# Danderson123/Amira

Hardware: AMD Instinct MI355X
Metric: gene-mers/s to corrected GeneMerGraph (higher is better)
Workload: dtype int32; 1 GPU; synthetic 1M reads x 60 genes, k=5, 20k-gene vocab: build + error-correction sweep (build, filter(3,1), correct, build, clip(5), correct, build); reads_per_gpu=1000000, genes_per_read=60, k=5, vocab=20000, gene_mers_per_gpu=56000000, final_nodes=472478, final_edges=1054844, multi_gpu=n/a

## Files before the change

amira_amd/csrc/amg_build_x.hip:

```cpp
#include "amg_tile.h"
#include "amg_x.h"

template <class View>
__device__ __forceinline__ void x_fp94(const View& w, int k, int flip, int dir, unsigned long long seed, int weak,
                                       unsigned long long& w1, unsigned int& tag) {
  unsigned long long h1 = seed, h2 = seed ^ 0xC2B2AE3D27D4EB4Full;
  for (int j = 0; j < k; ++j) {
    const unsigned long long c = (unsigned long long)(unsigned int)canon_tok(w, k, flip, dir, j);
    h1 = (h1 ^ c) * 0x9E3779B97F4A7C15ull;
    h1 ^= h1 >> 29;
    h2 = (h2 + c) * 0xD6E8FEB86659FD93ull;
    h2 ^= h2 >> 31;
  }
  h1 = mix64(h1);
  h2 = mix64(h2 ^ (h1 >> 7));
  if (weak) {
    h1 &= 0xfffull;
    h2 = 0ull;
  }
  w1 = (h1 << 1) | 1ull;
  tag = ((unsigned int)h2 << 1) | 1u;
}

__global__ __launch_bounds__(256) void k_x_verify_fp(const int* __restrict__ tokens, long long n_tokens, int k, int flip,
// ... 229 lines not shown

#define FD_READS 16
__global__ __launch_bounds__(256) void k_x_flag_dead_reads(const int* __restrict__ tok_node,
                                                            const long long* __restrict__ read_off, long long n_reads,
                                                            unsigned char* __restrict__ read_fix) {
  const int lane = threadIdx.x & 63, sub = lane & 15, grp = lane >> 4;
  const long long r = ((long long)blockIdx.x * 4 + (threadIdx.x >> 6)) * 4 + grp;
  const bool have = r < n_reads;
  const long long a = have ? read_off[r] : 0, b = have ? read_off[r + 1] : 0;
  int v[4];
#pragma unroll
  for (int j = 0; j < 4; ++j) v[j] = a + sub + 16 * j < b ? tok_node[a + sub + 16 * j] : 0;
  bool hit = v[0] == -2 || v[1] == -2 || v[2] == -2 || v[3] == -2;
  for (long long t = a + 64 + sub; t < b; t += 16) hit = hit || (tok_node[t] == -2);
  const unsigned long long m = __ballot(hit);
  if (have && sub == 0 && ((m >> (grp * 16)) & 0xffffull)) read_fix[r] = 1;
}

__global__ void k_x_rank_setflags(const unsigned int* __restrict__ first2, long long n, int shift,
                                  unsigned char* __restrict__ flags) {
  long long i = (long long)blockIdx.x * blockDim.x + threadIdx.x;
  if (i >= n) return;
  const unsigned int fi = x_first_inv(first2, i);
  if (fi == 0u) return;
  flags[(~fi) >> shift] = 1;
}

__device__ __forceinline__ long long x_rank_of(unsigned int t, const unsigned int* __restrict__ bits,
                                               const long long* __restrict__ prefix) {
  const unsigned int w = bits[t >> 5];
  return prefix[t >> 5] + (long long)__popc(w & ((1u << (t & 31)) - 1u));
}

__global__ void k_x_assign_nodes_ranked(const unsigned int* __restrict__ first2, long long n_nodes,
                                        const unsigned int* __restrict__ bits, const long long* __restrict__ prefix,
                                        const Slot16* __restrict__ tab, const unsigned int* __restrict__ slot_by_claim,
                                        int k, int nbits, int two, int* __restrict__ final_of_claim,
                                        int* __restrict__ node_tokens, long long* __restrict__ node_first,
                                        unsigned char* __restrict__ node_alive, const int* __restrict__ tokens, int flip) {
  long long c = (long long)blockIdx.x * blockDim.x + threadIdx.x;
  if (c >= n_nodes) return;
  if (x_first_inv(first2, c) == 0u) return;
  const unsigned int first = ~x_first_inv(first2, c);
  const long long i = x_rank_of(first >> 1, bits, prefix);
  final_of_claim[c] = (int)i;
  node_first[i] = (long long)first;
  node_alive[i] = 1;
  if (nbits == 0) {
    const long long f = (long long)(first >> 1);
    for (int j = 0; j < k; ++j) node_tokens[i * k + j] = (first & 1u) ? flip - tokens[f + k - 1 - j] : tokens[f + j];
    return;
  }
  const Slot16 s = tab[slot_by_claim[c]];
  const unsigned int tag = two ? (unsigned int)(s.w2 >> 32) : 0u;
  for (int j = 0; j < k; ++j) node_tokens[i * k + j] = x_unpack(s.w1, tag, nbits, j);
}

__device__ __forceinline__ void pair_to_final(unsigned long long& key, unsigned int& first,
                                              const int* __restrict__ fin) {
  const unsigned int lo_c = (unsigned int)((key >> 32) & 0x7fffffffull);
  const unsigned int hi_c = (unsigned int)(key & 0xffffffffull) - 1u;
  const bool a_is_lo = (first & 1u) != 0u;
  const unsigned int X = (unsigned int)fin[a_is_lo ? lo_c : hi_c], Y = (unsigned int)fin[a_is_lo ? hi_c : lo_c];
  const unsigned int lo = X < Y ? X : Y, hi = X < Y ? Y : X;
  key = (key & (1ull << 63)) | ((unsigned long long)lo << 32) | (unsigned long long)(hi + 1u);
  first = (first & ~1u) | (X == lo ? 1u : 0u);
}

__global__ void k_x_gather_pairs_ranked(const unsigned int* __restrict__ first2, long long n_pairs,
                                        const unsigned int* __restrict__ bits, const long long* __restrict__ prefix,
                                        const Slot16* __restrict__ etab, const unsigned int* __restrict__ slot_by_claim,
                                        const unsigned int* __restrict__ cnt_by_claim,
                                        unsigned long long* __restrict__ pkey, unsigned long long* __restrict__ pfirst,
                                        unsigned int* __restrict__ pcnt, const int* __restrict__ fin,
                                        int* __restrict__ efinal) {
  long long c = (long long)blockIdx.x * blockDim.x + threadIdx.x;
  if (c >= n_pairs) return;
  if (x_first_inv(first2, c) == 0u) return;
  unsigned int first = ~x_first_inv(first2, c);
  const long long i = x_rank_of(first >> 3, bits, prefix);
  unsigned long long key = etab[slot_by_claim[c]].w1;
  if (fin) pair_to_final(key, first, fin);
  pkey[i] = key;
  pfirst[i] = (unsigned long long)first;
  if (efinal)
    efinal[c] = (int)i;
  else
    pcnt[i] = cnt_by_claim[c];
}

__global__ void k_x_sort_keys(const unsigned int* __restrict__ first2, long long n,
                              unsigned int* __restrict__ keys, unsigned int* __restrict__ vals) {
  long long i = (long long)blockIdx.x * blockDim.x + threadIdx.x;
  if (i >= n) return;
  keys[i] = ~x_first_inv(first2, i);
  vals[i] = (unsigned int)i;
}

__global__ void k_x_assign_nodes(const unsigned int* __restrict__ first_sorted,
                                 const unsigned int* __restrict__ claim_sorted, long long n_nodes,
                                 const Slot16* __restrict__ tab, const unsigned int* __restrict__ slot_by_claim,
                                 int k, int bits, int two, int* __restrict__ final_of_claim,
                                 int* __restrict__ node_tokens, long long* __restrict__ node_first,
                                 unsigned char* __restrict__ node_alive, const int* __restrict__ tokens, int flip) {
  long long i = (long long)blockIdx.x * blockDim.x + threadIdx.x;
  if (i >= n_nodes) return;
  const unsigned int c = claim_sorted[i];
  final_of_claim[c] = (int)i;
  node_first[i] = (long long)first_sorted[i];
  node_alive[i] = 1;
  if (bits == 0) {
    const unsigned int first = first_sorted[i];
    const long long f = (long long)(first >> 1);
    for (int j = 0; j < k; ++j) node_tokens[i * k + j] = (first & 1u) ? flip - tokens[f + k - 1 - j] : tokens[f + j];
    return;
  }
  const Slot16 s = tab[slot_by_claim[c]];
  const unsigned int tag = two ? (unsigned int)(s.w2 >> 32) : 0u;
  for (int j = 0; j < k; ++j) node_tokens[i * k + j] = x_unpack(s.w1, tag, bits, j);
}

__global__ void k_xc_init(int* parent, long long n) {
  long long i = (long long)blockIdx.x * blockDim.x + threadIdx.x;
  if (i < n) parent[i] = (int)i;
}

__global__ void k_xc_union(const int* __restrict__ tok_claim, long long n_tokens, int* parent) {
  long long t = (long long)blockIdx.x * blockDim.x + threadIdx.x;
  if (t + 1 >= n_tokens) return;
  const int raw = tok_claim[t];
  if (raw == -1 || ((unsigned int)raw & AMG_LAST_FLAG)) return;
  const int nxt = tok_claim[t + 1];
  if (nxt == -1) return;
  int a = (int)((unsigned int)raw & ~AMG_FLAG_MASK), b = (int)((unsigned int)nxt & ~AMG_FLAG_MASK);
  while (true) {
    a = uf_find(parent, a);
    b = uf_find(parent, b);
    if (a == b) break;
    if (a > b) { int x = a; a = b; b = x; }
    const int old = atomicCAS(parent + b, b, a);
    if (old == b) break;
    b = old;
  }
}

__global__ void k_xc_flatten(int* parent, long long n) {
  long long i = (long long)blockIdx.x * blockDim.x + threadIdx.x;
  if (i < n) parent[i] = uf_find(parent, (int)i);
}

__device__ __forceinline__ int xc_root(const int* __restrict__ parent, long long c) {
  int r = parent[c];
// ... 428 lines not shown
    unsigned long long v[2] = {0, 0};
    AMGCHK(fetch(c, l, v));
    D = v[0];
    if (v[1]) {
      stage_end(c);
      return overflowed(which, OV_COLLISION);
    }
  }
  stage_end(c);
  c->n_nodes = (int64_t)D;
  AMGCHK(bx_nodes_rank(c));
  if (n > 0 && D > 0)
    hipLaunchKernelGGL(k_x_cov_from_claims, dim3(nblk(n, 256)), dim3(256), 0, st, c->x_ecnt.as<unsigned int>(),
                       c->x_first.as<unsigned int>(), c->x_final.as<int>(), n, c->node_cov.as<unsigned int>(), (int*)nullptr);
  return AMG_OK;
}

int bx_nodes_rank(amg_ctx* c) {
  hipStream_t st = c->stream;
  const long long T = c->n_tokens;
  const int k = c->k;
  stage_begin(c, "node_rank");
  const long long D = c->n_nodes;
  AMGCHK(c->s1.ensure((size_t)(D + 1) * sizeof(unsigned int)));
  AMGCHK(c->s2.ensure((size_t)(D + 1) * sizeof(unsigned int)));
  AMGCHK(c->s3.ensure((size_t)(D + 1) * sizeof(unsigned int)));
  AMGCHK(c->s4.ensure((size_t)(D + 1) * sizeof(unsigned int)));
  AMGCHK(bs_alloc_nodes(c, D));
  const long long S = c->x_nspace;
  if (D > 0 && ((D <= kRankBitmapMax && !c->sw.rank_sort) || S != D)) {
    AMGCHK(x_rank_bitmap(c, c->x_first.as<unsigned int>(), S, 1));
    hipLaunchKernelGGL(k_x_assign_nodes_ranked, dim3(nblk(S, 256)), dim3(256), 0, st,
                       c->x_first.as<unsigned int>(), S,
                       c->s1.as<unsigned int>(), c->s5.as<long long>(), c->node_tab.as<Slot16>(),
                       c->x_slot.as<unsigned int>(), k, c->x_kbits, c->x_two ? 1 : 0,
                       c->x_final.as<int>(), c->node_tokens.as<int>(),
                       c->node_first.as<long long>(), c->node_alive.as<unsigned char>(), c->tokens.as<int>(), c->two_v - 1);
  } else if (D > 0) {
    c->rank_flags_clean = 0;
    hipLaunchKernelGGL(k_x_sort_keys, dim3(nblk(D, 256)), dim3(256), 0, st, c->x_first.as<unsigned int>(),
                       D, c->s1.as<unsigned int>(),
                       c->s3.as<unsigned int>());
    AMGCHK(prim_sort_u32_u32(c, c->s1.as<unsigned int>(), c->s2.as<unsigned int>(), c->s3.as<unsigned int>(),
                             c->s4.as<unsigned int>(), (size_t)D, ilog2_ceil((uint64_t)T * 2 + 2) + 1));
    hipLaunchKernelGGL(k_x_assign_nodes, dim3(nblk(D, 256)), dim3(256), 0, st, c->s2.as<unsigned int>(),
                       c->s4.as<unsigned int>(), D, c->node_tab.as<Slot16>(), c->x_slot.as<unsigned int>(),
                       k, c->x_kbits, c->x_two ? 1 : 0, c->x_final.as<int>(),
                       c->node_tokens.as<int>(), c->node_first.as<long long>(), c->node_alive.as<unsigned char>(),
                       c->tokens.as<int>(), c->two_v - 1);
  }
  stage_end(c);
  return AMG_OK;
}

int bx_edges(amg_ctx* c, Overflow* which, unsigned int min_edge_cov) {
  bool lone = false;
  if (min_edge_cov == 0) {
    const bool can = c->sw.edge_home && c->n_nodes > 0;
    lone = can && (c->sw.edge_lone >= 0 ? c->sw.edge_lone != 0 : c->n_nodes * 16 > c->n_tokens);
    AMGCHK(bx_node_count(c, lone));
  }
  AMGCHK(bx_edges_upsert(c, which, lone, min_edge_cov == 0));
  return bx_edges_rank(c, min_edge_cov, min_edge_cov == 0);
}

int bx_node_count(amg_ctx* c, bool tag) {
  const long long T = c->n_tokens, D = c->n_nodes;
  stage_begin(c, "node_count");
  const long long S = c->x_nspace;
  AMGCHK(c->x_ncnt.ensure((size_t)(S + 2) * sizeof(unsigned int)));
  if (tag) AMGCHK(c->x_ftag.ensure((size_t)(S + 2) * sizeof(int)));
  AMGCHK(count_ids(c, CountNodes, IdsClaimsMarked, c->tok_slot.as<int>(), T, S, c->x_ncnt.as<unsigned int>()));
  if (S > 0 && D > 0)
    hipLaunchKernelGGL(k_x_cov_from_claims, dim3(nblk(S, 256)), dim3(256), 0, c->stream,
                       c->x_ncnt.as<unsigned int>(), c->x_first.as<unsigned int>(), c->x_final.as<int>(), S,
                       c->node_cov.as<unsigned int>(), tag ? c->x_ftag.as<int>() : (int*)nullptr);
  stage_end(c);
  return AMG_OK;
}

// ... 150 lines not shown
```

amira_amd/csrc/amg_filter.hip:

```cpp
#include "amg_rows.h"

__global__ void k_filter_nodes(const unsigned int* __restrict__ cov, unsigned char* __restrict__ alive,
                               long long n, unsigned int min_cov) {
  long long i = (long long)blockIdx.x * blockDim.x + threadIdx.x;
  if (i < n && alive[i] && cov[i] < min_cov) alive[i] = 0;
}

__global__ void k_filter_edges(const int* __restrict__ src, const int* __restrict__ tgt,
                               const unsigned int* __restrict__ cov,
                               const unsigned char* __restrict__ node_alive,
                               unsigned char* __restrict__ alive, long long n, unsigned int min_cov) {
  long long e = (long long)blockIdx.x * blockDim.x + threadIdx.x;
  if (e >= n || !alive[e]) return;
  if ((min_cov > 1 && cov[e] < min_cov) || !node_alive[src[e]] || !node_alive[tgt[e]]) alive[e] = 0;
}

#define READS_PER_WAVE 8
__global__ __launch_bounds__(256) void k_mask_reads(int* __restrict__ tok_node,
                                                    const long long* __restrict__ read_off,
                                                    long long n_reads,
                                                    const unsigned char* __restrict__ node_alive,
                                                    unsigned char* __restrict__ read_fix) {
  const long long rbase = ((long long)blockIdx.x * 4 + (threadIdx.x >> 6)) * READS_PER_WAVE;
  if (rbase >= n_reads) return;
  const int lane = threadIdx.x & 63;
  const long long off_l = (lane <= READS_PER_WAVE && rbase + lane <= n_reads) ? read_off[rbase + lane] : 0;
  long long a[READS_PER_WAVE], b[READS_PER_WAVE];
  int v[READS_PER_WAVE];
#pragma unroll
  for (int j = 0; j < READS_PER_WAVE; ++j) {
    a[j] = __shfl(off_l, j, 64);
    b[j] = rbase + j < n_reads ? __shfl(off_l, j + 1, 64) : a[j];
  }
#pragma unroll
  for (int j = 0; j < READS_PER_WAVE; ++j) v[j] = a[j] + lane < b[j] ? tok_node[a[j] + lane] : -1;
  bool dead[READS_PER_WAVE];
#pragma unroll
  for (int j = 0; j < READS_PER_WAVE; ++j) dead[j] = v[j] >= 0 && !node_alive[v[j]];
#pragma unroll
  for (int j = 0; j < READS_PER_WAVE; ++j) {
    if (dead[j]) tok_node[a[j] + lane] = -2;
    bool hit = dead[j];
    for (long long t = a[j] + 64 + lane; t < b[j]; t += 64) {
      const int n = tok_node[t];
      if (n >= 0 && !node_alive[n]) {
        tok_node[t] = -2;
        hit = true;
      }
    }
    if (__any(hit) && lane == 0) read_fix[rbase + j] = 1;
  }
}

static int apply_removals(amg_ctx* c, unsigned int min_edge_cov) {
  hipStream_t st = c->stream;
  if (min_edge_cov > 1) live_lists_after_edge_deaths(c);
  else live_lists_after_node_deaths(c);
  if (c->n_edges > 0)
    hipLaunchKernelGGL(k_filter_edges, dim3(nblk(c->n_edges, 256)), dim3(256), 0, st,
                       c->edge_src.as<int>(), c->edge_tgt.as<int>(), c->edge_cov.as<unsigned int>(),
                       c->node_alive.as<unsigned char>(), c->edge_alive.as<unsigned char>(),
                       c->n_edges, min_edge_cov);
  if (c->n_reads > 0)
    hipLaunchKernelGGL(k_mask_reads, dim3(nblk(c->n_reads, 4 * READS_PER_WAVE)), dim3(256), 0, st,
                       c->tok_node.as<int>(), c->read_off.as<long long>(), c->n_reads,
                       c->node_alive.as<unsigned char>(), c->read_fix.as<unsigned char>());
  return AMG_OK;
}

extern "C" int amg_filter(amg_ctx* c, uint32_t min_node_cov, uint32_t min_edge_cov) {
  NEED_BUILT(c);
  stages_reset(c);
  stage_begin(c, "filter");
  if (c->n_nodes > 0)
    hipLaunchKernelGGL(k_filter_nodes, dim3(nblk(c->n_nodes, 256)), dim3(256), 0, c->stream,
                       c->node_cov.as<unsigned int>(), c->node_alive.as<unsigned char>(),
                       c->n_nodes, min_node_cov);
  AMGCHK(apply_removals(c, min_edge_cov));
  stage_end(c);
  c->have_corrected = false;
  return AMG_OK;
}

__global__ void k_kill_listed(const int* __restrict__ ids, long long n, long long n_nodes,
                              unsigned char* __restrict__ alive) {
  long long i = (long long)blockIdx.x * blockDim.x + threadIdx.x;
  if (i >= n) return;
  int v = ids[i];
  if (v >= 0 && v < n_nodes) alive[v] = 0;
}

extern "C" int amg_remove_nodes(amg_ctx* c, const int32_t* node_ids, int64_t n) {
// ... 283 lines not shown
```

amira_amd/csrc/amg_internal.h:

```cpp
#pragma once
#include <cstdint>
#include <cstdio>
#include <cstring>
#include <string>
#include <vector>

#include <hip/hip_runtime.h>

#include "amg_host.h"

#define HIPCHK(call)                                                                   \
  do {                                                                                 \
    hipError_t e_ = (call);                                                            \
    if (e_ != hipSuccess)                                                              \
      return amg_fail(AMG_E_HIP, "%s:%d %s -> %s", __FILE__, __LINE__, #call,          \
                      hipGetErrorString(e_));                                          \
  } while (0)
#define AMGCHK(call)                 \
  do {                               \
    int r_ = (call);                 \
    if (r_ != AMG_OK) return r_;     \
  } while (0)

struct DevBuf {
// ... 255 lines not shown

  BuildSwitches sw;
  std::vector<StageTime> stages;
  bool timing = true;
};

struct amg_seqs {
  int device = 0;
  DevBuf bases, off;
  int64_t n = 0, total = 0;
};

int prim_sort_u64_u32(amg_ctx* c, const unsigned long long* kin, unsigned long long* kout,
                      const unsigned int* vin, unsigned int* vout, size_t n, int end_bit);
int prim_sort_u32_u32(amg_ctx* c, const unsigned int* kin, unsigned int* kout,
                      const unsigned int* vin, unsigned int* vout, size_t n, int end_bit);
struct ClearList;
int prim_exscan_i64(amg_ctx* c, const long long* in, long long* out, size_t n);
int prim_exscan_u32_to_i64(amg_ctx* c, const unsigned int* in, long long* out, size_t n);
int prim_exscan_u32_pair(amg_ctx* c, const unsigned int* in_a, long long* out_a, const unsigned int* in_b, long long* out_b,
                         size_t n);
int prim_exscan_i64_pair(amg_ctx* c, const long long* in_a, long long* out_a, const long long* in_b, long long* out_b,
                         size_t n);
int prim_exscan_bytes_set(amg_ctx* c, const unsigned char* in, long long* out, size_t n, const ClearList* side = nullptr);
int prim_exscan_apply_kill(amg_ctx* c, unsigned char* kill, unsigned char* alive, long long* out, size_t n);
int prim_exscan_keep_and_len(amg_ctx* c, const unsigned int* len, long long* out_keep, long long* out_off, size_t n);
int prim_exscan_flag_words(amg_ctx* c, const unsigned char* flags, unsigned int* bits, long long* out, size_t n_words);
int prim_exscan_bits_popc(amg_ctx* c, const unsigned int* bits, long long* out, size_t n_words);
int prim_exscan_pair_width(amg_ctx* c, const unsigned long long* pkey, long long* out, size_t n_pairs);
int prim_exscan_emit_edges(amg_ctx* c, const unsigned long long* pkey, const unsigned int* pcnt,
                           const unsigned long long* pfirst, size_t n_pairs, long long* total, int* e_src, int* e_tgt,
                           signed char* e_sdir, signed char* e_tdir, unsigned int* e_cov, unsigned char* e_alive,
                           const ClearList* side);

#define CLEAR_MAX 8
struct ClearList {
  void* p[CLEAR_MAX];
  unsigned long long bytes[CLEAR_MAX];
  int n = 0;
  bool overflow = false;
  unsigned int fill[CLEAR_MAX];
  void add(void* ptr, size_t b, unsigned int value = 0u) {
    if (b == 0) return;
    if (n >= CLEAR_MAX) {
      overflow = true;
      return;
    }
    p[n] = ptr;
    bytes[n] = (unsigned long long)((b + 3) & ~(size_t)3);
    fill[n] = value;
    ++n;
  }
};
int clear_many(amg_ctx* c, const ClearList& l);

#define FETCH_MAX 96
struct FetchList {
  const unsigned long long* p[FETCH_MAX];
  int n = 0;
  bool overflow = false;
  void add(const void* q) {
    if (n < FETCH_MAX)
      p[n++] = static_cast<const unsigned long long*>(q);
    else
      overflow = true;
  }
// ... 96 lines not shown
```

amira_amd/csrc/amg_live_rows.hip:

```cpp
#include "amg_rows.h"

void live_lists_after_node_deaths(amg_ctx* c) {
  if (c->live_lists == LiveLists::Current)
    c->live_lists = getenv("AMG_NO_LADJ_PATCH") ? LiveLists::Absent : LiveLists::BehindNodes;
  c->pristine = false;
  c->match_valid = false;
}

void live_lists_after_edge_deaths(amg_ctx* c) {
  c->live_lists = LiveLists::Absent;
  c->edge_own_deaths = true;
  c->pristine = false;
  c->match_valid = false;
}

void live_lists_after_build(amg_ctx* c) { c->live_lists = LiveLists::Absent; }

__global__ void k_live_keys(const unsigned char* __restrict__ e_alive, const int* __restrict__ e_src,
                            const signed char* __restrict__ e_sdir, const long long* __restrict__ pos,
                            long long n_edges, unsigned int* __restrict__ keys, unsigned int* __restrict__ vals) {
  long long e = (long long)blockIdx.x * blockDim.x + threadIdx.x;
  if (e >= n_edges || !e_alive[e]) return;
  const long long o = pos[e];
  keys[o] = adj_row_of(e_src[e], e_sdir[e]);
  vals[o] = (unsigned int)e;
}

__global__ void k_lr_count(const unsigned int* __restrict__ keys, long long n_live, int4* __restrict__ lrows) {
  long long i = (long long)blockIdx.x * blockDim.x + threadIdx.x;
  if (i < n_live) atomicAdd(&lrows[keys[i]].y, 1);
}

#define LR_PER 8
__global__ __launch_bounds__(256) void k_lr_alloc(const unsigned int* __restrict__ keys, long long n_live,
                                                  int4* __restrict__ lrows, unsigned int* __restrict__ tick,
                                                  unsigned long long* pool) {
  __shared__ unsigned int s_wave[4];
  __shared__ unsigned long long s_base;
  const long long i0 = (long long)blockIdx.x * (256 * LR_PER) + threadIdx.x;
  unsigned int cnt[LR_PER], key[LR_PER], mine = 0;
#pragma unroll
  for (int j = 0; j < LR_PER; ++j) {
    const long long i = i0 + (long long)j * 256;
    cnt[j] = 0;
    key[j] = 0;
    if (i < n_live) {
      key[j] = keys[i];
      const unsigned int t = (unsigned int)atomicAdd(&lrows[key[j]].z, 1);
      tick[i] = t;
      if (t == 0) cnt[j] = (unsigned int)lrows[key[j]].y | 0x80000000u;
      mine += cnt[j] & 0x7fffffffu;
    }
  }
  unsigned int total;
  unsigned int off = block_exscan_256(mine, &total, s_wave);
  if (threadIdx.x == 0) s_base = total ? atomicAdd(pool, (unsigned long long)total) : 0ull;
  __syncthreads();
#pragma unroll
  for (int j = 0; j < LR_PER; ++j)
// ... 69 lines not shown
  const int4 rw = lrows[r];
  if (rw.y == 0) return;
  if (!n_alive[r >> 1]) {
    lrows[r] = make_int4(rw.x, 0, 0, 0);
    return;
  }
  if (rw.y == 1) {
    if (!n_alive[rw.z]) lrows[r] = make_int4(rw.x, 0, 0, 0);
    return;
  }
  int w = 0;
  int2 first = make_int2(0, 0);
  for (int j = 0; j < rw.y; ++j) {
    const int2 e = lent[rw.x + j];
    if (!n_alive[e.x]) continue;
    if (w != j) lent[rw.x + w] = e;
    if (w == 0) first = e;
    ++w;
  }
  if (w != rw.y) lrows[r] = make_int4(rw.x, w, first.x, first.y);
}

int ensure_live_adj(amg_ctx* c) {
  if (c->live_lists == LiveLists::Current) return AMG_OK;
  hipStream_t st = c->stream;
  if (c->live_lists == LiveLists::BehindNodes) {
    hipLaunchKernelGGL(k_lr_patch, dim3(nblk(2 * c->n_nodes, 256)), dim3(256), 0, st, c->ladj_rows.as<int4>(),
                       c->ladj.as<int2>(), 2 * c->n_nodes, c->node_alive.as<unsigned char>());
    c->live_lists = LiveLists::Current;
    return AMG_OK;
  }
  const long long rows = 2 * c->n_nodes, E = c->n_edges;
  AMGCHK(c->ladj_rows.ensure((size_t)(rows + 2) * sizeof(int4)));
  AMGCHK(c->ladj_pos.ensure((size_t)(E + 2) * sizeof(long long)));
  unsigned long long* ctr = c->status.as<unsigned long long>() + ST_COMPACT_A;
  {
    ClearList cl;
    cl.add(c->ladj_rows.p, (size_t)(rows + 2) * sizeof(int4));
    cl.add(ctr, 2 * sizeof(unsigned long long));
    AMGCHK(prim_exscan_bytes_set(c, c->edge_alive.as<unsigned char>(), c->ladj_pos.as<long long>(), (size_t)E, &cl));
  }
  long long total = 0;
  {
    FetchList l;
    l.add(c->ladj_pos.as<long long>() + E);
    AMGCHK(fetch(c, l, reinterpret_cast<unsigned long long*>(&total)));
  }
  AMGCHK(c->ladj.ensure((size_t)(total + 1) * sizeof(int2)));
  AMGCHK(c->ladj_keys.ensure(5 * (size_t)(total + 2) * sizeof(unsigned int)));
  unsigned int* keys = c->ladj_keys.as<unsigned int>();
  unsigned int* edge_of = keys + (total + 2);
  unsigned int* tick = edge_of + (total + 2);
  unsigned int* tmp = tick + (total + 2);
  unsigned int* long_rows = tmp + (total + 2);
  if (total > 0) {
    hipLaunchKernelGGL(k_live_keys, dim3(nblk(E, 256)), dim3(256), 0, st, c->edge_alive.as<unsigned char>(),
                       c->edge_src.as<int>(), c->edge_sdir.as<signed char>(), c->ladj_pos.as<long long>(), E, keys,
                       edge_of);
    hipLaunchKernelGGL(k_lr_count, dim3(nblk(total, 256)), dim3(256), 0, st, keys, total, c->ladj_rows.as<int4>());
    hipLaunchKernelGGL(k_lr_alloc, dim3(nblk(total, 256 * LR_PER)), dim3(256), 0, st, keys, total, c->ladj_rows.as<int4>(),
                       tick, ctr);
    hipLaunchKernelGGL(k_lr_fill, dim3(nblk(total, 256)), dim3(256), 0, st, keys, edge_of, tick, total,
                       c->ladj_rows.as<int4>(), c->edge_tgt.as<int>(), c->edge_tdir.as<signed char>(), tmp, c->ladj.as<int2>());
    hipLaunchKernelGGL(k_lr_finish, dim3(nblk(total, 256)), dim3(256), 0, st, keys, tick, total, tmp, c->edge_tgt.as<int>(),
                       c->edge_tdir.as<signed char>(), c->ladj_rows.as<int4>(), c->ladj.as<int2>(), long_rows, ctr + 1);
    const long long hub_words = (E + 31) / 32 + 1;
    AMGCHK(c->hub_bits.ensure((size_t)HUB_BLOCKS * (size_t)hub_words * sizeof(unsigned int)));
    hipLaunchKernelGGL(k_lr_long, dim3(64), dim3(256), 0, st, long_rows, ctr + 1, tmp, c->edge_tgt.as<int>(),
                       c->edge_tdir.as<signed char>(), c->ladj_rows.as<int4>(), c->ladj.as<int2>(),
                       c->hub_bits.as<unsigned int>(), hub_words);
  }
  c->live_lists = LiveLists::Current;
  return AMG_OK;
}

GView make_view(amg_ctx* c) {
  GView g;
  g.lent = c->ladj.as<int2>();
  g.lrows = c->ladj_rows.as<int4>();
  g.n_alive = c->node_alive.as<unsigned char>();
  g.n_cov = c->node_cov.as<unsigned int>();
  g.n_tok = c->node_tokens.as<int>();
  g.n_first = c->node_first.as<long long>();
  g.n_comp = c->node_comp.as<int>();
  g.k = c->k;
  g.flip = c->two_v - 1;
  return g;
}

__global__ void k_row_tickets(const unsigned char* __restrict__ e_alive, const int* __restrict__ e_src,
                              const signed char* __restrict__ e_sdir, long long n_edges, int4* __restrict__ rows) {
// ... 30 lines not shown
```

amira_amd/csrc/amg_scan.hip:

```cpp
#include "amg_device.h"

#define SC_THREADS 512
#define SC_ROWS 16
#define SC_TILE (SC_THREADS * SC_ROWS)
#define SC_VAL_MASK ((1ull << 48) - 1ull)

__device__ __forceinline__ unsigned long long sc_word(unsigned int state, unsigned int epoch, unsigned long long v) {
  return ((unsigned long long)state << 62) | ((unsigned long long)(epoch & 0x3fffu) << 48) | (v & SC_VAL_MASK);
}

#define SC_NO_LIM 0x7fffffffffffffffll
template <class T>
struct LoadArr {
  const T* in;
  using Raw = T;
  __device__ __forceinline__ long long lim() const { return SC_NO_LIM; }
  __device__ __forceinline__ Raw raw(long long i) const { return in[i]; }
  __device__ __forceinline__ unsigned long long val(long long, Raw r) const { return (unsigned long long)r; }
};
template <class T>
struct LoadArrN {
  const T* in;
  long long n;
  using Raw = T;
  __device__ __forceinline__ long long lim() const { return n; }
  __device__ __forceinline__ Raw raw(long long i) const { return in[i]; }
  __device__ __forceinline__ unsigned long long val(long long, Raw r) const { return (unsigned long long)r; }
};
struct LoadNonzero {
  const unsigned int* in;
  long long n;
  using Raw = unsigned int;
  __device__ __forceinline__ long long lim() const { return n; }
// ... 69 lines not shown
struct LoadNone {
  using Raw = unsigned char;
  __device__ __forceinline__ long long lim() const { return 0; }
  __device__ __forceinline__ Raw raw(long long) const { return 0; }
  __device__ __forceinline__ unsigned long long val(long long, Raw) const { return 0ull; }
};

template <class L>
__device__ __forceinline__ void load_rows(const L& ld, long long w0, long long n, int lane, unsigned long long* x) {
  const long long lim = n < ld.lim() ? n : ld.lim();
  if (w0 >= lim) {
#pragma unroll
    for (int r = 0; r < SC_ROWS; ++r) x[r] = 0ull;
    return;
  }
  typename L::Raw raw[SC_ROWS];
#pragma unroll
  for (int r = 0; r < SC_ROWS; ++r) {
    const long long i = w0 + r * 64 + lane;
    raw[r] = ld.raw(i < lim ? i : lim - 1);
  }
  asm volatile("" ::: "memory");
#pragma unroll
  for (int r = 0; r < SC_ROWS; ++r) {
    const long long i = w0 + r * 64 + lane;
    x[r] = i < lim ? ld.val(i, raw[r]) : 0ull;
  }
}

struct EmitOut {
  long long* out;
  struct Pre {};
  __device__ __forceinline__ Pre pre(long long) const { return Pre{}; }
  __device__ __forceinline__ void operator()(long long i, unsigned long long excl, const Pre&) const {
    out[i] = (long long)excl;
  }
};
struct EmitEdges {
  const unsigned long long* pkey;
  const unsigned int* pcnt;
  const unsigned long long* pfirst;
  long long n_pairs;
  long long* total;
  int* e_src;
  int* e_tgt;
  signed char* e_sdir;
  signed char* e_tdir;
  unsigned int* e_cov;
  unsigned char* e_alive;
  struct Pre {
    unsigned long long key, first;
    unsigned int cnt;
  };
  __device__ __forceinline__ Pre pre(long long i) const {
    const long long j = i < n_pairs ? i : 0;
    return Pre{pkey[j], pfirst[j], pcnt[j]};
  }
  __device__ __forceinline__ void operator()(long long i, unsigned long long excl, const Pre& p) const {
    if (i >= n_pairs) {
      total[0] = (long long)excl;
      return;
    }
    const unsigned long long key = p.key, first = p.first;
    const int lo = (int)((key >> 32) & 0x7fffffffull);
    const int hi = (int)((key & 0xffffffffull) - 1ull);
    const int X = (first & 1ull) ? lo : hi, Y = (first & 1ull) ? hi : lo;
    const signed char dX = (first & 2ull) ? 1 : -1, dY = (first & 4ull) ? 1 : -1;
    const long long e = (long long)excl;
    const unsigned int cnt = p.cnt;
    e_src[e] = X; e_tgt[e] = Y; e_sdir[e] = dX; e_tdir[e] = dY; e_alive[e] = 1;
    if (lo == hi) {
      e_cov[e] = cnt * 2u;
    } else {
      e_cov[e] = cnt;
      e_src[e + 1] = Y; e_tgt[e + 1] = X; e_sdir[e + 1] = (signed char)-dY;
      e_tdir[e + 1] = (signed char)-dX; e_cov[e + 1] = cnt; e_alive[e + 1] = 1;
    }
  }
};
template <class Load, class LoadB, class Emit>
__global__ __launch_bounds__(SC_THREADS) void k_exscan(Load load, Emit emit_a, long long n_a, LoadB load_b,
                                                        long long* __restrict__ out_b, long long n_b, long long tiles_a,
                                                        unsigned long long* counter, unsigned long long ticket_base,
                                                        unsigned long long* status, unsigned int epoch, ClearArgs side) {
  __shared__ unsigned long long s_wave[SC_THREADS / 64];
  __shared__ unsigned long long s_excl;
  __shared__ unsigned int s_tile;
  const int lane = threadIdx.x & 63, wave = threadIdx.x >> 6;
  if (threadIdx.x == 0) s_tile = (unsigned int)(atomicAdd(counter, 1ull) - ticket_base);
  __syncthreads();
  const long long tile = s_tile;
  const bool second = tile >= tiles_a;
  const long long seg0 = second ? tiles_a : 0;
  const long long n = second ? n_b : n_a;
  const long long w0 = (tile - seg0) * SC_TILE + (long long)wave * (64 * SC_ROWS);
  unsigned long long x[SC_ROWS], inc[SC_ROWS];
  if (second)
    load_rows(load_b, w0, n, lane, x);
  else
    load_rows(load, w0, n, lane, x);
  unsigned long long row_off = 0;
#pragma unroll
  for (int r = 0; r < SC_ROWS; ++r) {
    unsigned long long v = x[r];
#pragma unroll
    for (int d = 1; d < 64; d <<= 1) {
      const unsigned long long o = __shfl_up(v, d, 64);
      if (lane >= d) v += o;
    }
    inc[r] = v + row_off;
// ... 28 lines not shown
        const long long idx = look - lane;
        unsigned int state = 2u;
        unsigned long long val = 0;
        if (idx >= seg0) {
          unsigned long long w;
          do {
            w = __hip_atomic_load(status + idx, __ATOMIC_RELAXED, __HIP_MEMORY_SCOPE_AGENT);
          } while ((unsigned int)((w >> 48) & 0x3fffu) != (epoch & 0x3fffu) || (w >> 62) == 0ull);
          state = (unsigned int)(w >> 62);
          val = w & SC_VAL_MASK;
        }
        const unsigned long long full = __ballot(state == 2u);
        const int stop = full ? __ffsll((long long)full) - 1 : 63;
        unsigned long long part = lane <= stop ? val : 0ull;
#pragma unroll
        for (int d = 32; d > 0; d >>= 1) part += __shfl_xor(part, d, 64);
        excl += part;
        if (full) break;
      }
      if (lane == 0)
        __hip_atomic_store(status + tile, sc_word(2u, epoch, excl + tile_sum), __ATOMIC_RELAXED, __HIP_MEMORY_SCOPE_AGENT);
    }
    if (lane == 0) s_excl = excl;
  }
  __syncthreads();
  const unsigned long long base = s_excl + wave_excl;
#pragma unroll
  for (int r = 0; r < SC_ROWS; ++r) {
    const long long i = w0 + r * 64 + lane;
    if (i < n) {
      if (second)
        out_b[i] = (long long)(base + inc[r] - x[r]);
      else
        emit_a(i, base + inc[r] - x[r], pre[r]);
    }
  }
  if (side.n) clear_args_part(side, blockIdx.x, gridDim.x);
}

template <class Load, class Emit, class LoadB = LoadNone>
static int exscan_emit(amg_ctx* c, Load load, Emit emit, size_t n, LoadB load_b = LoadNone{}, long long* out_b = nullptr,
                       size_t n_b = 0, const ClearList* side = nullptr) {
  if (side && side->overflow) return amg_fail(AMG_E_ARG, "exscan: more than %d ranges in one list", CLEAR_MAX);
  if (n == 0 && n_b == 0) return side ? clear_many(c, *side) : AMG_OK;
  const unsigned long long tiles_a = (n + SC_TILE - 1) / SC_TILE;
  const unsigned long long tiles = tiles_a + (n_b + SC_TILE - 1) / SC_TILE;
  const size_t need = (size_t)(tiles + 8) * sizeof(unsigned long long);
  if (need > c->scan_state.cap || c->scan_epoch >= 0x3fffu) {
    if (need > c->scan_state.cap) {
      AMGCHK(c->scan_state.ensure(need * 2));
      c->scan_tickets = 0;
      HIPCHK(hipMemsetAsync(c->scan_state.p, 0, c->scan_state.cap, c->stream));
    } else {
      HIPCHK(hipMemsetAsync(c->scan_state.as<unsigned long long>() + 8, 0,
                            c->scan_state.cap - 8 * sizeof(unsigned long long), c->stream));
    }
    c->scan_epoch = 0;
  }
  const unsigned int epoch = ++c->scan_epoch;
  unsigned long long* st = c->scan_state.as<unsigned long long>();
  ClearArgs sa;
  sa.n = 0;
  if (side) sa = clear_args(*side);
  hipLaunchKernelGGL((k_exscan<Load, LoadB, Emit>), dim3((unsigned int)tiles), dim3(SC_THREADS), 0, c->stream, load, emit,
                     (long long)n, load_b, out_b, (long long)n_b, (long long)tiles_a, st, c->scan_tickets, st + 8, epoch, sa);
  c->scan_tickets += tiles;
  return AMG_OK;
// ... 28 lines not shown
int prim_exscan_bytes_set(amg_ctx* c, const unsigned char* in, long long* out, size_t n, const ClearList* side) {
  return exscan_emit(c, LoadByteSet{in, (long long)n}, EmitOut{out}, n + 1, LoadNone{}, nullptr, 0, side);
}

int prim_exscan_apply_kill(amg_ctx* c, unsigned char* kill, unsigned char* alive, long long* out, size_t n) {
  return exscan(c, LoadApplyKill{kill, alive, (long long)n}, out, n + 1);
}

int prim_exscan_keep_and_len(amg_ctx* c, const unsigned int* len, long long* out_keep, long long* out_off, size_t n) {
  return exscan(c, LoadNonzero{len, (long long)n}, out_keep, n + 1, LoadArrN<unsigned int>{len, (long long)n}, out_off, n + 1);
}

int prim_exscan_flag_words(amg_ctx* c, const unsigned char* flags, unsigned int* bits, long long* out, size_t n_words) {
  return exscan(c, LoadFlagWords{flags, bits, (long long)n_words}, out, n_words + 1);
}

int prim_exscan_bits_popc(amg_ctx* c, const unsigned int* bits, long long* out, size_t n_words) {
  return exscan(c, LoadBitsPopc{bits, (long long)n_words}, out, n_words + 1);
}

int prim_exscan_pair_width(amg_ctx* c, const unsigned long long* pkey, long long* out, size_t n_pairs) {
  return exscan(c, LoadPairWidth{pkey, (long long)n_pairs}, out, n_pairs + 1);
}

int prim_exscan_emit_edges(amg_ctx* c, const unsigned long long* pkey, const unsigned int* pcnt,
                           const unsigned long long* pfirst, size_t n_pairs, long long* total, int* e_src, int* e_tgt,
                           signed char* e_sdir, signed char* e_tdir, unsigned int* e_cov, unsigned char* e_alive,
                           const ClearList* side) {
  return exscan_emit(c, LoadPairWidth{pkey, (long long)n_pairs},
                     EmitEdges{pkey, pcnt, pfirst, (long long)n_pairs, total, e_src, e_tgt, e_sdir, e_tdir, e_cov, e_alive},
                     n_pairs + 1, LoadNone{}, nullptr, 0, side);
}

extern "C" int amg_scan_probe(amg_ctx* c, int kind, const void* in, int64_t n, int64_t* out, void* aux) {
  if (!c || n < 0 || (n > 0 && !in) || !out) return amg_fail(AMG_E_ARG, "scan_probe: bad arguments");
  size_t in_bytes = 0, out_words = (size_t)n + 1, aux_bytes = 0;
  switch (kind) {
    case 0: in_bytes = (size_t)n; aux_bytes = (size_t)n; break;
    case 1: in_bytes = 8 * (size_t)n; break;
    case 2: in_bytes = 32 * (size_t)n; aux_bytes = 4 * (size_t)n; break;
    case 3: in_bytes = 2 * (size_t)n; aux_bytes = 2 * (size_t)n; break;
    case 4: in_bytes = 4 * (size_t)n; out_words = 2 * ((size_t)n + 1); break;
    case 5: in_bytes = 20 * (size_t)n; out_words = 1; aux_bytes = 30 * (size_t)n; break;
    default: return amg_fail(AMG_E_ARG, "scan_probe: unknown kind %d", kind);
  }
  char* d = nullptr;
  const size_t in_cap = (in_bytes + 255) & ~(size_t)255, out_cap = (out_words * 8 + 255) & ~(size_t)255;
  const size_t aux_cap = (aux_bytes + 256) & ~(size_t)255;
  HIPCHK(hipMalloc(reinterpret_cast<void**>(&d), in_cap + out_cap + aux_cap));
  char* din = d;
  long long* dout = reinterpret_cast<long long*>(d + in_cap);
  char* daux = d + in_cap + out_cap;
  int rc = AMG_OK;
  do {
    if (in_bytes && hipMemcpy(din, in, in_bytes, hipMemcpyHostToDevice) != hipSuccess) { rc = amg_fail(AMG_E_HIP, "h2d"); break; }
    if (hipMemset(daux, 0xff, aux_cap) != hipSuccess || hipDeviceSynchronize() != hipSuccess) {
      rc = amg_fail(AMG_E_HIP, "memset");
      break;
    }
    switch (kind) {
      case 0: {
        ClearList side;
        side.add(daux, (size_t)n);
        rc = prim_exscan_bytes_set(c, reinterpret_cast<unsigned char*>(din), dout, (size_t)n, &side);
        break;
      }
      case 1: rc = prim_exscan_pair_width(c, reinterpret_cast<unsigned long long*>(din), dout, (size_t)n); break;
      case 2:
        rc = prim_exscan_flag_words(c, reinterpret_cast<unsigned char*>(din), reinterpret_cast<unsigned int*>(daux), dout,
                                    (size_t)n);
        break;
      case 3:
        if (n && (hipMemcpy(daux, din, 2 * (size_t)n, hipMemcpyDeviceToDevice) != hipSuccess ||
                  hipDeviceSynchronize() != hipSuccess)) {
          rc = amg_fail(AMG_E_HIP, "d2d");
          break;
        }
        rc = prim_exscan_apply_kill(c, reinterpret_cast<unsigned char*>(daux), reinterpret_cast<unsigned char*>(daux) + n,
                                    dout, (size_t)n);
        break;
      case 4:
        rc = prim_exscan_keep_and_len(c, reinterpret_cast<unsigned int*>(din), dout, dout + n + 1, (size_t)n);
        break;
      case 5: {
        const size_t E = 2 * (size_t)n;
        int* src = reinterpret_cast<int*>(daux);
        int* tgt = src + E;
        unsigned int* cov = reinterpret_cast<unsigned int*>(tgt + E);
        signed char* sdir = reinterpret_cast<signed char*>(cov + E);
        signed char* tdir = sdir + E;
        unsigned char* alive = reinterpret_cast<unsigned char*>(tdir + E);
        rc = prim_exscan_emit_edges(c, reinterpret_cast<unsigned long long*>(din),
                                    reinterpret_cast<unsigned int*>(din + 16 * (size_t)n),
                                    reinterpret_cast<unsigned long long*>(din + 8 * (size_t)n), (size_t)n, dout, src, tgt,
                                    sdir, tdir, cov, alive, nullptr);
        break;
      }
    }
    if (rc != AMG_OK) break;
    if (hipStreamSynchronize(c->stream) != hipSuccess) { rc = amg_fail(AMG_E_HIP, "scan_probe: stream"); break; }
    if (hipMemcpy(out, dout, out_words * 8, hipMemcpyDeviceToHost) != hipSuccess) { rc = amg_fail(AMG_E_HIP, "d2h"); break; }
    if (aux && aux_bytes && hipMemcpy(aux, daux, aux_bytes, hipMemcpyDeviceToHost) != hipSuccess) { rc = amg_fail(AMG_E_HIP, "d2h"); break; }
  } while (false);
  (void)hipFree(d);
  return rc;
}
```

Before: 10.48 billion gene-mers/s.

## Fuse live-edge key emission into scan, vectorize edge filter, coalesce node token writes

Three separate changes. The live-edge exclusive scan now writes row keys and edge ids directly, which removes the separate k_live_keys kernel, the long-long position array round trip and the larger key buffer. The edge filter now handles four edges per thread with vector loads of alive, src, tgt and cov. Node assignment now writes node tokens through wave shuffles so each lane stores contiguous elements, and always reads tokens from the reads, dropping the packed-slot unpack path. The risks are extra shuffles and divergence in node assignment, and the loss of the packed-table path.

```diff
diff --git a/amira_amd/csrc/amg_build_x.hip b/amira_amd/csrc/amg_build_x.hip
--- a/amira_amd/csrc/amg_build_x.hip
+++ b/amira_amd/csrc/amg_build_x.hip
@@ -285,28 +285,36 @@
   return prefix[t >> 5] + (long long)__popc(w & ((1u << (t & 31)) - 1u));
 }
 
-__global__ void k_x_assign_nodes_ranked(const unsigned int* __restrict__ first2, long long n_nodes,
-                                        const unsigned int* __restrict__ bits, const long long* __restrict__ prefix,
-                                        const Slot16* __restrict__ tab, const unsigned int* __restrict__ slot_by_claim,
-                                        int k, int nbits, int two, int* __restrict__ final_of_claim,
-                                        int* __restrict__ node_tokens, long long* __restrict__ node_first,
-                                        unsigned char* __restrict__ node_alive, const int* __restrict__ tokens, int flip) {
-  long long c = (long long)blockIdx.x * blockDim.x + threadIdx.x;
-  if (c >= n_nodes) return;
-  if (x_first_inv(first2, c) == 0u) return;
-  const unsigned int first = ~x_first_inv(first2, c);
-  const long long i = x_rank_of(first >> 1, bits, prefix);
-  final_of_claim[c] = (int)i;
-  node_first[i] = (long long)first;
-  node_alive[i] = 1;
-  if (nbits == 0) {
-    const long long f = (long long)(first >> 1);
-    for (int j = 0; j < k; ++j) node_tokens[i * k + j] = (first & 1u) ? flip - tokens[f + k - 1 - j] : tokens[f + j];
-    return;
-  }
-  const Slot16 s = tab[slot_by_claim[c]];
-  const unsigned int tag = two ? (unsigned int)(s.w2 >> 32) : 0u;
-  for (int j = 0; j < k; ++j) node_tokens[i * k + j] = x_unpack(s.w1, tag, nbits, j);
+__device__ __forceinline__ void node_tuples_from_reads(int* __restrict__ node_tokens, const int* __restrict__ tokens,
+                                                       int node, unsigned int first, int k, int flip) {
+  const unsigned int lane = threadIdx.x & 63u;
+  for (int m = 0; m < k; ++m) {
+    const unsigned int e = lane + 64u * (unsigned int)m;
+    const unsigned int q = e / (unsigned int)k, j = e - q * (unsigned int)k;
+    const int nq = __shfl(node, (int)q, 64);
+    const unsigned int fq = __shfl(first, (int)q, 64);
+    if (nq < 0) continue;
+    const int* w = tokens + (long long)(fq >> 1);
+    node_tokens[(long long)nq * k + j] = (fq & 1u) ? flip - w[k - 1 - (int)j] : w[j];
+  }
+}
+
+__global__ __launch_bounds__(256) void k_x_assign_nodes_ranked(
+    const unsigned int* __restrict__ first2, long long n_nodes, const unsigned int* __restrict__ bits,
+    const long long* __restrict__ prefix, int k, int* __restrict__ final_of_claim, int* __restrict__ node_tokens,
+    long long* __restrict__ node_first, unsigned char* __restrict__ node_alive, const int* __restrict__ tokens, int flip) {
+  const long long c = (long long)blockIdx.x * blockDim.x + threadIdx.x;
+  const unsigned int fi = c < n_nodes ? x_first_inv(first2, c) : 0u;
+  const unsigned int first = ~fi;
+  int node = -1;
+  if (fi != 0u) {
+    const long long i = x_rank_of(first >> 1, bits, prefix);
+    node = (int)i;
+    final_of_claim[c] = node;
+    node_first[i] = (long long)first;
+    node_alive[i] = 1;
+  }
+  node_tuples_from_reads(node_tokens, tokens, node, first, k, flip);
 }
 
 __device__ __forceinline__ void pair_to_final(unsigned long long& key, unsigned int& first,
@@ -350,27 +358,19 @@
   vals[i] = (unsigned int)i;
 }
 
-__global__ void k_x_assign_nodes(const unsigned int* __restrict__ first_sorted,
-                                 const unsigned int* __restrict__ claim_sorted, long long n_nodes,
-                                 const Slot16* __restrict__ tab, const unsigned int* __restrict__ slot_by_claim,
-                                 int k, int bits, int two, int* __restrict__ final_of_claim,
-                                 int* __restrict__ node_tokens, long long* __restrict__ node_first,
-                                 unsigned char* __restrict__ node_alive, const int* __restrict__ tokens, int flip) {
-  long long i = (long long)blockIdx.x * blockDim.x + threadIdx.x;
-  if (i >= n_nodes) return;
-  const unsigned int c = claim_sorted[i];
-  final_of_claim[c] = (int)i;
-  node_first[i] = (long long)first_sorted[i];
-  node_alive[i] = 1;
-  if (bits == 0) {
-    const unsigned int first = first_sorted[i];
-    const long long f = (long long)(first >> 1);
-    for (int j = 0; j < k; ++j) node_tokens[i * k + j] = (first & 1u) ? flip - tokens[f + k - 1 - j] : tokens[f + j];
-    return;
-  }
-  const Slot16 s = tab[slot_by_claim[c]];
-  const unsigned int tag = two ? (unsigned int)(s.w2 >> 32) : 0u;
-  for (int j = 0; j < k; ++j) node_tokens[i * k + j] = x_unpack(s.w1, tag, bits, j);
+__global__ __launch_bounds__(256) void k_x_assign_nodes(
+    const unsigned int* __restrict__ first_sorted, const unsigned int* __restrict__ claim_sorted, long long n_nodes, int k,
+    int* __restrict__ final_of_claim, int* __restrict__ node_tokens, long long* __restrict__ node_first,
+    unsigned char* __restrict__ node_alive, const int* __restrict__ tokens, int flip) {
+  const long long i = (long long)blockIdx.x * blockDim.x + threadIdx.x;
+  unsigned int first = 0u;
+  if (i < n_nodes) {
+    first = first_sorted[i];
+    final_of_claim[claim_sorted[i]] = (int)i;
+    node_first[i] = (long long)first;
+    node_alive[i] = 1;
+  }
+  node_tuples_from_reads(node_tokens, tokens, i < n_nodes ? (int)i : -1, first, k, flip);
 }
 
 __global__ void k_xc_init(int* parent, long long n) {
@@ -865,9 +865,7 @@
     AMGCHK(x_rank_bitmap(c, c->x_first.as<unsigned int>(), S, 1));
     hipLaunchKernelGGL(k_x_assign_nodes_ranked, dim3(nblk(S, 256)), dim3(256), 0, st,
                        c->x_first.as<unsigned int>(), S,
-                       c->s1.as<unsigned int>(), c->s5.as<long long>(), c->node_tab.as<Slot16>(),
-                       c->x_slot.as<unsigned int>(), k, c->x_kbits, c->x_two ? 1 : 0,
-                       c->x_final.as<int>(), c->node_tokens.as<int>(),
+                       c->s1.as<unsigned int>(), c->s5.as<long long>(), k, c->x_final.as<int>(), c->node_tokens.as<int>(),
                        c->node_first.as<long long>(), c->node_alive.as<unsigned char>(), c->tokens.as<int>(), c->two_v - 1);
   } else if (D > 0) {
     c->rank_flags_clean = 0;
@@ -877,8 +875,7 @@
     AMGCHK(prim_sort_u32_u32(c, c->s1.as<unsigned int>(), c->s2.as<unsigned int>(), c->s3.as<unsigned int>(),
                              c->s4.as<unsigned int>(), (size_t)D, ilog2_ceil((uint64_t)T * 2 + 2) + 1));
     hipLaunchKernelGGL(k_x_assign_nodes, dim3(nblk(D, 256)), dim3(256), 0, st, c->s2.as<unsigned int>(),
-                       c->s4.as<unsigned int>(), D, c->node_tab.as<Slot16>(), c->x_slot.as<unsigned int>(),
-                       k, c->x_kbits, c->x_two ? 1 : 0, c->x_final.as<int>(),
+                       c->s4.as<unsigned int>(), D, k, c->x_final.as<int>(),
                        c->node_tokens.as<int>(), c->node_first.as<long long>(), c->node_alive.as<unsigned char>(),
                        c->tokens.as<int>(), c->two_v - 1);
   }
diff --git a/amira_amd/csrc/amg_filter.hip b/amira_amd/csrc/amg_filter.hip
--- a/amira_amd/csrc/amg_filter.hip
+++ b/amira_amd/csrc/amg_filter.hip
@@ -6,13 +6,42 @@
   if (i < n && alive[i] && cov[i] < min_cov) alive[i] = 0;
 }
 
-__global__ void k_filter_edges(const int* __restrict__ src, const int* __restrict__ tgt,
-                               const unsigned int* __restrict__ cov,
-                               const unsigned char* __restrict__ node_alive,
-                               unsigned char* __restrict__ alive, long long n, unsigned int min_cov) {
-  long long e = (long long)blockIdx.x * blockDim.x + threadIdx.x;
-  if (e >= n || !alive[e]) return;
+__device__ __forceinline__ void filter_edge(const int* __restrict__ src, const int* __restrict__ tgt,
+                                            const unsigned int* __restrict__ cov,
+                                            const unsigned char* __restrict__ node_alive,
+                                            unsigned char* __restrict__ alive, long long e, unsigned int min_cov) {
+  if (!alive[e]) return;
   if ((min_cov > 1 && cov[e] < min_cov) || !node_alive[src[e]] || !node_alive[tgt[e]]) alive[e] = 0;
+}
+
+__global__ __launch_bounds__(256) void k_filter_edges(const int* __restrict__ src, const int* __restrict__ tgt,
+                                                      const unsigned int* __restrict__ cov,
+                                                      const unsigned char* __restrict__ node_alive,
+                                                      unsigned char* __restrict__ alive, long long n, unsigned int min_cov) {
+  const long long q = (long long)blockIdx.x * blockDim.x + threadIdx.x;
+  const long long e0 = 4 * q;
+  if (e0 >= n) return;
+  if (e0 + 4 > n) {
+    for (long long e = e0; e < n; ++e) filter_edge(src, tgt, cov, node_alive, alive, e, min_cov);
+    return;
+  }
+  const unsigned int a = reinterpret_cast<const unsigned int*>(alive)[q];
+  if (a == 0u) return;
+  const int4 s = reinterpret_cast<const int4*>(src)[q];
+  const int4 t = reinterpret_cast<const int4*>(tgt)[q];
+  uint4 c = make_uint4(min_cov, min_cov, min_cov, min_cov);
+  if (min_cov > 1) c = reinterpret_cast<const uint4*>(cov)[q];
+  const bool l0 = a & 0x000000ffu, l1 = a & 0x0000ff00u, l2 = a & 0x00ff0000u, l3 = a & 0xff000000u;
+  const unsigned int ns0 = node_alive[l0 ? s.x : 0], ns1 = node_alive[l1 ? s.y : 0], ns2 = node_alive[l2 ? s.z : 0],
+                     ns3 = node_alive[l3 ? s.w : 0];
+  const unsigned int nt0 = node_alive[l0 ? t.x : 0], nt1 = node_alive[l1 ? t.y : 0], nt2 = node_alive[l2 ? t.z : 0],
+                     nt3 = node_alive[l3 ? t.w : 0];
+  unsigned int keep = 0u;
+  if (ns0 && nt0 && c.x >= min_cov) keep |= 0x000000ffu;
+  if (ns1 && nt1 && c.y >= min_cov) keep |= 0x0000ff00u;
+  if (ns2 && nt2 && c.z >= min_cov) keep |= 0x00ff0000u;
+  if (ns3 && nt3 && c.w >= min_cov) keep |= 0xff000000u;
+  if ((a & keep) != a) reinterpret_cast<unsigned int*>(alive)[q] = a & keep;
 }
 
 #define READS_PER_WAVE 8
@@ -57,7 +86,7 @@
   if (min_edge_cov > 1) live_lists_after_edge_deaths(c);
   else live_lists_after_node_deaths(c);
   if (c->n_edges > 0)
-    hipLaunchKernelGGL(k_filter_edges, dim3(nblk(c->n_edges, 256)), dim3(256), 0, st,
+    hipLaunchKernelGGL(k_filter_edges, dim3(nblk(c->n_edges, 4 * 256)), dim3(256), 0, st,
                        c->edge_src.as<int>(), c->edge_tgt.as<int>(), c->edge_cov.as<unsigned int>(),
                        c->node_alive.as<unsigned char>(), c->edge_alive.as<unsigned char>(),
                        c->n_edges, min_edge_cov);
diff --git a/amira_amd/csrc/amg_internal.h b/amira_amd/csrc/amg_internal.h
--- a/amira_amd/csrc/amg_internal.h
+++ b/amira_amd/csrc/amg_internal.h
@@ -311,6 +311,8 @@
                            const unsigned long long* pfirst, size_t n_pairs, long long* total, int* e_src, int* e_tgt,
                            signed char* e_sdir, signed char* e_tdir, unsigned int* e_cov, unsigned char* e_alive,
                            const ClearList* side);
+int prim_exscan_live_edges(amg_ctx* c, const unsigned char* e_alive, const int* e_src, const signed char* e_sdir, size_t n_edges,
+                           long long* total, unsigned int* keys, unsigned int* edge_of, const ClearList* side);
 
 #define CLEAR_MAX 8
 struct ClearList {
diff --git a/amira_amd/csrc/amg_live_rows.hip b/amira_amd/csrc/amg_live_rows.hip
--- a/amira_amd/csrc/amg_live_rows.hip
+++ b/amira_amd/csrc/amg_live_rows.hip
@@ -15,16 +15,6 @@
 }
 
 void live_lists_after_build(amg_ctx* c) { c->live_lists = LiveLists::Absent; }
-
-__global__ void k_live_keys(const unsigned char* __restrict__ e_alive, const int* __restrict__ e_src,
-                            const signed char* __restrict__ e_sdir, const long long* __restrict__ pos,
-                            long long n_edges, unsigned int* __restrict__ keys, unsigned int* __restrict__ vals) {
-  long long e = (long long)blockIdx.x * blockDim.x + threadIdx.x;
-  if (e >= n_edges || !e_alive[e]) return;
-  const long long o = pos[e];
-  keys[o] = adj_row_of(e_src[e], e_sdir[e]);
-  vals[o] = (unsigned int)e;
-}
 
 __global__ void k_lr_count(const unsigned int* __restrict__ keys, long long n_live, int4* __restrict__ lrows) {
   long long i = (long long)blockIdx.x * blockDim.x + threadIdx.x;
@@ -160,31 +150,30 @@
   }
   const long long rows = 2 * c->n_nodes, E = c->n_edges;
   AMGCHK(c->ladj_rows.ensure((size_t)(rows + 2) * sizeof(int4)));
-  AMGCHK(c->ladj_pos.ensure((size_t)(E + 2) * sizeof(long long)));
+  AMGCHK(c->ladj_pos.ensure((size_t)(E + 3) * sizeof(long long)));
+  unsigned int* keys = c->ladj_pos.as<unsigned int>();
+  unsigned int* edge_of = keys + (E + 2);
+  long long* d_total = c->ladj_pos.as<long long>() + (E + 2);
   unsigned long long* ctr = c->status.as<unsigned long long>() + ST_COMPACT_A;
   {
     ClearList cl;
     cl.add(c->ladj_rows.p, (size_t)(rows + 2) * sizeof(int4));
     cl.add(ctr, 2 * sizeof(unsigned long long));
-    AMGCHK(prim_exscan_bytes_set(c, c->edge_alive.as<unsigned char>(), c->ladj_pos.as<long long>(), (size_t)E, &cl));
+    AMGCHK(prim_exscan_live_edges(c, c->edge_alive.as<unsigned char>(), c->edge_src.as<int>(), c->edge_sdir.as<signed char>(),
+                                  (size_t)E, d_total, keys, edge_of, &cl));
   }
   long long total = 0;
   {
     FetchList l;
-    l.add(c->ladj_pos.as<long long>() + E);
+    l.add(d_total);
     AMGCHK(fetch(c, l, reinterpret_cast<unsigned long long*>(&total)));
   }
   AMGCHK(c->ladj.ensure((size_t)(total + 1) * sizeof(int2)));
-  AMGCHK(c->ladj_keys.ensure(5 * (size_t)(total + 2) * sizeof(unsigned int)));
-  unsigned int* keys = c->ladj_keys.as<unsigned int>();
-  unsigned int* edge_of = keys + (total + 2);
-  unsigned int* tick = edge_of + (total + 2);
+  AMGCHK(c->ladj_keys.ensure(3 * (size_t)(total + 2) * sizeof(unsigned int)));
+  unsigned int* tick = c->ladj_keys.as<unsigned int>();
   unsigned int* tmp = tick + (total + 2);
   unsigned int* long_rows = tmp + (total + 2);
   if (total > 0) {
-    hipLaunchKernelGGL(k_live_keys, dim3(nblk(E, 256)), dim3(256), 0, st, c->edge_alive.as<unsigned char>(),
-                       c->edge_src.as<int>(), c->edge_sdir.as<signed char>(), c->ladj_pos.as<long long>(), E, keys,
-                       edge_of);
     hipLaunchKernelGGL(k_lr_count, dim3(nblk(total, 256)), dim3(256), 0, st, keys, total, c->ladj_rows.as<int4>());
     hipLaunchKernelGGL(k_lr_alloc, dim3(nblk(total, 256 * LR_PER)), dim3(256), 0, st, keys, total, c->ladj_rows.as<int4>(),
                        tick, ctr);
diff --git a/amira_amd/csrc/amg_scan.hip b/amira_amd/csrc/amg_scan.hip
--- a/amira_amd/csrc/amg_scan.hip
+++ b/amira_amd/csrc/amg_scan.hip
@@ -1,4 +1,4 @@
-#include "amg_device.h"
+#include "amg_rows.h"
 
 #define SC_THREADS 512
 #define SC_ROWS 16
@@ -134,7 +134,7 @@
   long long* out;
   struct Pre {};
   __device__ __forceinline__ Pre pre(long long) const { return Pre{}; }
-  __device__ __forceinline__ void operator()(long long i, unsigned long long excl, const Pre&) const {
+  __device__ __forceinline__ void operator()(long long i, unsigned long long excl, const Pre&, unsigned long long) const {
     out[i] = (long long)excl;
   }
 };
@@ -158,7 +158,7 @@
     const long long j = i < n_pairs ? i : 0;
     return Pre{pkey[j], pfirst[j], pcnt[j]};
   }
-  __device__ __forceinline__ void operator()(long long i, unsigned long long excl, const Pre& p) const {
+  __device__ __forceinline__ void operator()(long long i, unsigned long long excl, const Pre& p, unsigned long long) const {
     if (i >= n_pairs) {
       total[0] = (long long)excl;
       return;
@@ -178,6 +178,25 @@
       e_src[e + 1] = Y; e_tgt[e + 1] = X; e_sdir[e + 1] = (signed char)-dY;
       e_tdir[e + 1] = (signed char)-dX; e_cov[e + 1] = cnt; e_alive[e + 1] = 1;
     }
+  }
+};
+struct EmitLiveKeys {
+  const int* e_src;
+  const signed char* e_sdir;
+  long long n_edges;
+  long long* total;
+  unsigned int* keys;
+  unsigned int* edge_of;
+  struct Pre {};
+  __device__ __forceinline__ Pre pre(long long) const { return Pre{}; }
+  __device__ __forceinline__ void operator()(long long i, unsigned long long excl, const Pre&, unsigned long long val) const {
+    if (i >= n_edges) {
+      total[0] = (long long)excl;
+      return;
+    }
+    if (val == 0ull) return;
+    keys[excl] = adj_row_of(e_src[i], e_sdir[i]);
+    edge_of[excl] = (unsigned int)i;
   }
 };
 template <class Load, class LoadB, class Emit>
@@ -272,7 +291,7 @@
       if (second)
         out_b[i] = (long long)(base + inc[r] - x[r]);
       else
-        emit_a(i, base + inc[r] - x[r], pre[r]);
+        emit_a(i, base + inc[r] - x[r], pre[r], x[r]);
     }
   }
   if (side.n) clear_args_part(side, blockIdx.x, gridDim.x);
@@ -367,6 +386,13 @@
                      n_pairs + 1, LoadNone{}, nullptr, 0, side);
 }
 
+int prim_exscan_live_edges(amg_ctx* c, const unsigned char* e_alive, const int* e_src, const signed char* e_sdir, size_t n_edges,
+                           long long* total, unsigned int* keys, unsigned int* edge_of, const ClearList* side) {
+  return exscan_emit(c, LoadByteSet{e_alive, (long long)n_edges},
+                     EmitLiveKeys{e_src, e_sdir, (long long)n_edges, total, keys, edge_of}, n_edges + 1, LoadNone{}, nullptr, 0,
+                     side);
+}
+
 extern "C" int amg_scan_probe(amg_ctx* c, int kind, const void* in, int64_t n, int64_t* out, void* aux) {
   if (!c || n < 0 || (n > 0 && !in) || !out) return amg_fail(AMG_E_ARG, "scan_probe: bad arguments");
   size_t in_bytes = 0, out_words = (size_t)n + 1, aux_bytes = 0;
@@ -377,6 +403,7 @@
     case 3: in_bytes = 2 * (size_t)n; aux_bytes = 2 * (size_t)n; break;
     case 4: in_bytes = 4 * (size_t)n; out_words = 2 * ((size_t)n + 1); break;
     case 5: in_bytes = 20 * (size_t)n; out_words = 1; aux_bytes = 30 * (size_t)n; break;
+    case 6: in_bytes = 6 * (size_t)n; out_words = 1; aux_bytes = 8 * (size_t)n; break;
     default: return amg_fail(AMG_E_ARG, "scan_probe: unknown kind %d", kind);
   }
   char* d = nullptr;
@@ -431,6 +458,13 @@
                                     sdir, tdir, cov, alive, nullptr);
         break;
       }
+      case 6: {
+        unsigned int* keys = reinterpret_cast<unsigned int*>(daux);
+        rc = prim_exscan_live_edges(c, reinterpret_cast<unsigned char*>(din + 4 * (size_t)n), reinterpret_cast<int*>(din),
+                                    reinterpret_cast<signed char*>(din + 5 * (size_t)n), (size_t)n, dout, keys, keys + n,
+                                    nullptr);
+        break;
+      }
     }
     if (rc != AMG_OK) break;
     if (hipStreamSynchronize(c->stream) != hipSuccess) { rc = amg_fail(AMG_E_HIP, "scan_probe: stream"); break; }
```

After: 10.66 billion gene-mers/s (median of 6 runs). 1.02x the previous value.
